# craabreu/openmm-nonbonded-slicing

Hardware: AMD Instinct MI355X
Metric: ns/day (force evaluation only, dt = 2 fs) (higher is better)
Workload: dtype f32

## Files before the change

### openmm-nonbonded-slicing_amd/csrc/engine.hip

```cpp
#include "../../include/snb.h"
#include "snb_internal.h"
#include "switches.h"
#include "host_lists.h"
#include "ewald_fit.h"

#include <algorithm>
#include <cstdio>
#include <cstdlib>
#include <chrono>
#include <cmath>
#include <cstring>
#include <map>
#include <numeric>
#include <set>
#include <thread>
#include <tuple>
#include <type_traits>

namespace snb {

static thread_local std::string g_createError;

static inline void cpuRelax() {
#if defined(__x86_64__) || defined(__i386__)
// ... 902 lines not shown
            if (!noSortGraph && !sortGraphBroken && !cfg.disable_graph && !sortGraphSuspect && !plainSort && N <= (1 << 20)) {
                hipGraphExec_t sortGraphExec = nullptr;
                for (auto& g : sortGraphs) if (g.key.size() == sizeof(key) && std::memcmp(g.key.data(), &key, sizeof(key)) == 0) sortGraphExec = g.exec;
                if (!sortGraphExec) {
                    hipGraph_t graph = nullptr;
                    if (hipStreamBeginCapture(stream, hipStreamCaptureModeThreadLocal) == hipSuccess) {
                        bool threw = false;
                        try { launchNeighborSort<Real>(p, devUserPos, posIsDouble, posStride4, dSortTemp.p, tempBytes, stream); }
                        catch (...) { threw = true; }
                        hipError_t endErr = hipStreamEndCapture(stream, &graph);
                        if (threw) { endErr = hipErrorUnknown; (void)hipGetLastError(); }
                        if (endErr == hipSuccess && graph && hipGraphInstantiate(&sortGraphExec, graph, nullptr, nullptr, 0) == hipSuccess) {
                            SortGraph g; g.key.assign(reinterpret_cast<const unsigned char*>(&key), reinterpret_cast<const unsigned char*>(&key) + sizeof(key)); g.exec = sortGraphExec;
                            if (sortGraphs.size() < 4) sortGraphs.push_back(g);
                            else { (void)hipGraphExecDestroy(sortGraphs[sortGraphVictim].exec); sortGraphs[sortGraphVictim] = g; sortGraphVictim = (sortGraphVictim + 1) % 4; }
                        } else { sortGraphExec = nullptr; sortGraphBroken = true; (void)hipGetLastError(); }
                        if (graph) (void)hipGraphDestroy(graph);
                    } else { sortGraphBroken = true; (void)hipGetLastError(); }
                }
                if (sortGraphExec) { HIPCHECK(hipGraphLaunch(sortGraphExec, stream)); replayed = true; }
            }
            if (!replayed) launchNeighborSort<Real>(p, devUserPos, posIsDouble, posStride4, dSortTemp.p, tempBytes, stream);
        }
        HIPCHECK(hipEventRecord(evRebuild[2], stream));
        const bool predicted = npadPredict > 0 && !sw.nbSyncPadded;
        if (predicted) Npad = npadPredict;
        else {
            int npadDev = 0;
            HIPCHECK(hipMemcpyAsync(&npadDev, dCounters.p + 7, sizeof(int), hipMemcpyDeviceToHost, stream));
            HIPCHECK(hipStreamSynchronize(stream));
            if (npadDev < N || (npadDev & 31)) throw HipError{"neighbour build: inconsistent padded atom count"};
            Npad = npadDev;
        }
        numBlocks = Npad / 32;
        if (Npad >= (1 << SNB_JSHIFT_BITS) - 1) throw HipError{"too many atoms for the 25-bit tile index"};
        posq.resize(Npad); sigeps.resize(Npad); imageOffset.resize((size_t)3 * Npad);
        dSortedToUser.resize(Npad); atomSubset.resize(Npad); atomGrid.resize(Npad); blockSubset.resize(numBlocks);
        layoutForces();
        dBlockCenter.resize((size_t)3 * numBlocks); dBlockHalf.resize((size_t)3 * numBlocks);
        if (tileCap < (size_t)numBlocks * 40) tileCap = (size_t)numBlocks * 40;
        if (tileCap < 64 * 128) tileCap = 64 * 128;
        float sortMs = 0;
        if (!predicted) HIPCHECK(hipEventElapsedTime(&sortMs, evRebuild[0], evRebuild[2]));
        for (int attempt = 0; attempt < 3; attempt++) {
            tileJ.resize(tileCap * 32); tileInfo.resize(tileCap); masks.resize(tileCap * 32); workItems.resize(2 * (tileCap / 4 + 2 * numBlocks + 64)); workItemsStage.resize(tileCap / 4 + 2 * numBlocks + 64); workItemsPartial.resize(tileCap / 4 + 2 * numBlocks + 64);
            p.nPadded = Npad; p.nBlocks = numBlocks; p.blockSubset = blockSubset.p;
            p.shardBegin = shardBegin; p.shardWidth = shardEnd - shardBegin; p.shardPeriod = shardPeriod;
            p.exactPrune = sw.boxPrune ? 0 : 1; p.itemTiles = sw.itemTiles;
            p.blockCenter = dBlockCenter.p; p.blockHalf = dBlockHalf.p;
            p.sortedToUser = dSortedToUser.p; p.userToSorted = dUserToSorted.p; p.posq = posq.p; p.sigeps = sigeps.p; p.imageOffset = imageOffset.p;
            p.atomSubset = atomSubset.p; p.atomGrid = atomGrid.p; p.colRange = colRange.p; p.zIndex = dZIndex.p;
            dAtomCell.resize(Npad); p.atomCell = dAtomCell.p;
            const bool nbTrace = sw.nbTrace;
            if (nbTrace) { dNbTrace.resize((size_t)4 * numBlocks); p.dbgOut = dNbTrace.p; }
            p.tileJ = tileJ.p; p.tileInfo = tileInfo.p; p.masks = masks.p; p.workItems = workItems.p; p.workItemsStage = workItemsStage.p; p.workItemsPartial = workItemsPartial.p; p.counters = dCounters.p;
            p.tileCapacity = (int)tileCap; p.workCapacity = (int)(tileCap / 4 + 2 * numBlocks + 64); p.maskCapacity = (int)tileCap;
            if (!predicted || attempt > 0) HIPCHECK(hipEventRecord(evRebuild[0], stream));
            launchNeighborBuild<Real>(p, stream);
            HIPCHECK(hipEventRecord(evRebuild[1], stream));
            if (sideBuilding) {
                sideSeq = ++nbPubSeq;
                launchNeighborPublish(dCounters.p, dNbPub, sideSeq, stream);
                return true;
            }
            int h[8] = {0, 0, 0, 0, 0, 0, 0, 0};
            if (hNbPub && dNbPub && !sw.nbNoSpin) {
                const int seq = ++nbPubSeq;
                launchNeighborPublish(dCounters.p, dNbPub, seq, stream);
                waitForTotals(seq, h, stream);
                HIPCHECK(hipStreamSynchronize(stream));
            } else {
                HIPCHECK(hipMemcpyAsync(h, dCounters.p, sizeof(h), hipMemcpyDeviceToHost, stream));
                HIPCHECK(hipStreamSynchronize(stream));
            }
            if (!sortGraphSuspect && stats.n_rebuilds > 0 && h[7] > 2 * std::max(Npad, N) && !sideBuilding) {
                sortGraphSuspect = true;
                if (sw.verbose) fprintf(stderr, "[snb] rebuild: padded count %d after %d: phase A once more without its graph\n", h[7], Npad);
                return gpuRebuild();
            }
            if (predicted && (h[7] > Npad || h[7] < N || (h[7] & 31))) {
                if (h[7] < N || (h[7] & 31)) throw HipError{"neighbour build: inconsistent padded atom count"};
                npadPredict = 0; padMispredictions++;
                if (sw.verbose) fprintf(stderr, "[snb] rebuild: padded count %d exceeded the predicted %d, repeating with the exact count (%lld so far)\n", h[7], Npad, (long long)padMispredictions);
                return gpuRebuild();
            }
            if (nbTrace && h[3] == 0) {
                std::vector<long long> tr((size_t)4 * numBlocks);
                HIPCHECK(hipMemcpy(tr.data(), dNbTrace.p, sizeof(long long) * tr.size(), hipMemcpyDeviceToHost));
                long long t0min = tr[0], t1max = tr[1]; std::vector<long long> dur(numBlocks);
                tr.resize((size_t)4 * numBlocks);
                for (int b = 0; b < numBlocks; b++) { t0min = std::min(t0min, tr[2 * b]); t1max = std::max(t1max, tr[2 * b + 1]); dur[b] = tr[2 * b + 1] - tr[2 * b]; }
                std::vector<long long> sorted = dur; std::sort(sorted.begin(), sorted.end());
                fprintf(stderr, "[snb] nb trace: span %.1f us; per-block duration median %.1f us, p90 %.1f, p99 %.1f, max %.1f us; last start at %.1f us\n", (t1max - t0min) / 100.0, sorted[numBlocks / 2] / 100.0,
                        sorted[numBlocks * 9 / 10] / 100.0, sorted[numBlocks * 99 / 100] / 100.0, sorted.back() / 100.0, (t1max - t0min) / 100.0);
                { std::vector<long long> a(numBlocks), b(numBlocks), c(numBlocks);
                  for (int k = 0; k < numBlocks; k++) { a[k] = tr[2 * numBlocks + 2 * k] - tr[2 * k]; b[k] = tr[2 * numBlocks + 2 * k + 1] - tr[2 * numBlocks + 2 * k]; c[k] = tr[2 * k + 1] - tr[2 * numBlocks + 2 * k + 1]; }
                  std::sort(a.begin(), a.end()); std::sort(b.begin(), b.end()); std::sort(c.begin(), c.end());
                  fprintf(stderr, "[snb] nb trace: median prologue %.1f us, gather %.1f us, final flush %.1f us\n", a[numBlocks / 2] / 100.0, b[numBlocks / 2] / 100.0, c[numBlocks / 2] / 100.0); }
                long long lastStart = 0; for (int b = 0; b < numBlocks; b++) lastStart = std::max(lastStart, tr[2 * b] - t0min);
                fprintf(stderr, "[snb] nb trace: last block start %.1f us after the first\n", lastStart / 100.0);
            }
            if (h[3] == 0) { acceptBuild(h, sortMs); gpuBuilt = true; needRebuild = false; paramsDirty = false; stepsSinceRebuild = 0; (void)t0; return true; }
            if (sw.verbose) fprintf(stderr, "[snb] gpu neighbour build attempt %d: tiles %d work %d masks %d overflow %d partial %d maxPartTiles %d maxPartWork %d (cap %zu, region %zu / %zu)\n", attempt, h[0], h[1], h[2], h[3], h[4], h[5], h[6], tileCap, tileCap / 64, (tileCap / 4 + 2 * numBlocks + 64) / 64);
            if ((size_t)h[5] > tileCap / 64 || (size_t)h[6] > (tileCap / 4 + 2 * numBlocks + 64) / 64) { tileCap = std::max((size_t)h[5] * 64 * 5 / 4, tileCap * 3 / 2) + 4096; continue; }
            return false;
        }
        return false;
    }

    void fillPme(PmeParams<Real>& p, PmePlan<Real>& plan, bool wantEnergy, const int* need, bool cellsReady = false, bool trace = false) {
        p.d = plan.d; p.nsub = nGrids; p.natoms = Npad; p.posq = posq.p; p.sigeps = sigeps.p; p.atomSubset = atomSubset.p; p.atomGrid = atomGrid.p;
        p.cells = pmeCells.p;
        if (sw.pmeTrace) { if (!dPmeTrace.p) { dPmeTrace.resize(8); HIPCHECK(hipMemset(dPmeTrace.p, 0, 64)); } p.trace = dPmeTrace.p; }
        p.stepTrace = (trace && plan.dispersion == (cfg.method == SNB_LJPME)) ? dStepTrace.p : nullptr;
        p.cellsReady = (!plan.dispersion && cellsReady) ? 1 : 0;
        p.fixDev = dFixScale.p ? dFixScale.p + (plan.dispersion ? 2 : 0) : nullptr;
        p.gridReal = plan.gridReal.p; p.gridCplx = plan.gridCplx.p; p.planeB = plan.gridCplxB.p; p.planeEterm = plan.planeEtermReady ? plan.planeEterm.p : nullptr; p.twx = plan.twx.p; p.twy = plan.twy.p; p.twz = plan.twz.p;
        p.modx = plan.modx.p; p.mody = plan.mody.p; p.modz = plan.modz.p;
        const double det = box[0] * box[4] * box[8], sc = 1.0 / det;
        const double r[9] = {box[4] * box[8] * sc, 0, 0, -box[3] * box[8] * sc, box[0] * box[8] * sc, 0,
                             (box[3] * box[7] - box[4] * box[6]) * sc, -box[0] * box[7] * sc, box[0] * box[4] * sc};
        for (int i = 0; i < 9; i++) { p.recip[i] = (Real)r[i]; p.recipLo[i] = (Real)(r[i] - (double)p.recip[i]); }
        p.alpha = (Real)plan.alpha; p.volume = (Real)det; p.dispersion = plan.dispersion ? 1 : 0;
        p.lambdas = dLambdas.p; p.sliceNeed = need; p.gridSubset = gridSubset.p; p.nsubTotal = nsub; p.mix = cfg.shard_count == 1 ? 1 : 0;
        p.mix16 = sw.mix16 ? 1 : 0;
        p.sliceE = sliceE.p; p.fpx = fpx.p; p.fpy = fpy.p; p.fpz = fpz.p; p.wantEnergy = wantEnergy ? 1 : 0;
        p.sortNcx = p.sortNcy = 0; p.groupX = p.groupY = 1; p.colRange = nullptr;
        p.zSlabs = 1;
        if (plan.d.nz % 2 == 0 && plan.d.nz >= 32 && !(sizeof(Real) == 4)) p.zSlabs = 2;
        if (sw.zSlabs >= 1 && plan.d.nz % sw.zSlabs == 0) p.zSlabs = sw.zSlabs;
        int ncx, ncy, gx, gy;
        if (brickGeometry(plan, ncx, ncy, gx, gy)) {
            p.sortNcx = ncx; p.sortNcy = ncy; p.groupX = gx; p.groupY = gy; p.colRange = colRange.p;
            p.ownSlabs = plan.ownSlabs; p.ownMargin = plan.ownMargin; p.ownPartial = plan.ownPartial.p; p.ownBusy = plan.ownBusy.p;
            p.strays = plan.strays.p; p.strayCount = dStrayCount.p ? dStrayCount.p + (plan.dispersion ? 1 : 0) : nullptr;
            if (!p.ownPartial || !p.ownBusy || !p.strays || !p.strayCount) p.ownSlabs = 0;
        }
    }
    bool brickGeometry(const PmePlan<Real>& plan, int& ncx, int& ncy, int& gx, int& gy) const {
        if (colCells[0] <= 0) return false;
        ncx = pme.d.nx / colCells[0]; ncy = pme.d.ny / colCells[1];
        const int gMin = sw.brickGroup;
        auto group = [gMin](int n, int ncols) { if (n % ncols) return 0; const int cpc = n / ncols; for (int g = gMin; g <= 4; g++) if (g * cpc >= 5 && ncols % g == 0) return g; return 0; };
        gx = group(plan.d.nx, ncx); gy = group(plan.d.ny, ncy);
        const bool packable = plan.d.nx < 1024 && plan.d.ny < 1024 && plan.d.nz < 1024;
        return packable && gx > 0 && gy > 0 && sizeof(double) * (size_t)(gx * plan.d.nx / ncx) * (gy * plan.d.ny / ncy) * plan.d.nz <= 100 * 1024;
    }
    void planPlaneTable(PmePlan<Real>& plan) {
        if (!plan.planeEterm.p || !plan.gridCplxB.p || nGrids <= 0) { plan.planeEtermReady = false; return; }
        double key[10]; for (int i = 0; i < 9; i++) key[i] = box[i]; key[9] = plan.alpha;
        if (plan.planeEtermReady && plan.planeEtermFilled && std::memcmp(key, plan.planeEtermKey, sizeof(key)) == 0) return;
        std::memcpy(plan.planeEtermKey, key, sizeof(key));
        plan.planeEtermReady = false;
// ... 968 lines not shown
```

### openmm-nonbonded-slicing_amd/csrc/neighbor.hip

```cpp
#include "snb_internal.h"
#include <cstring>
#include <algorithm>
#include <string.h>
#include <rocprim/rocprim.hpp>

namespace snb {

struct Lattice { float ax, bx, by, cx, cy, cz; };
template <typename P> __device__ inline bool useBoxWalk(const P& p) { return p.boxWalk != 0; }
template <typename Real> __device__ inline Lattice latticeOf(const NbParams<Real>& p) {
    return Lattice{(float)p.boxm[0], (float)p.boxm[3], (float)p.boxm[4], (float)p.boxm[6], (float)p.boxm[7], (float)p.boxm[8]};
}
__device__ inline void minImage(float& dx, float& dy, float& dz, const Lattice& L) {
    float s = rintf(dz / L.cz); dx -= s * L.cx; dy -= s * L.cy; dz -= s * L.cz;
    s = rintf(dy / L.by); dx -= s * L.bx; dy -= s * L.by;
    s = rintf(dx / L.ax); dx -= s * L.ax;
}
__device__ inline int orderedInt(float f) { const int i = __float_as_int(f); return i >= 0 ? i : i ^ 0x7FFFFFFF; }
template <typename In> __global__ void k_nbExtent(const In* __restrict__ userPos, int stride, int n, int* __restrict__ ext) {
    const int u = blockIdx.x * blockDim.x + threadIdx.x;
    float lo[3] = {3e38f, 3e38f, 3e38f}, hi[3] = {-3e38f, -3e38f, -3e38f};
    if (u < n) for (int d = 0; d < 3; d++) { const float v = (float)userPos[(size_t)u * stride + d]; lo[d] = v; hi[d] = v; }
#pragma unroll
    for (int o = 32; o > 0; o >>= 1)
// ... 139 lines not shown
    if (b >= p.nBlocks) return;
    const int s = b * 32 + k;
    const bool real = p.sortedToUser[s] >= 0;
    const auto v = p.posq[s];
    float mn[3] = {real ? (float)v.x : 3e38f, real ? (float)v.y : 3e38f, real ? (float)v.z : 3e38f};
    float mx[3] = {real ? (float)v.x : -3e38f, real ? (float)v.y : -3e38f, real ? (float)v.z : -3e38f};
#pragma unroll
    for (int o = 16; o > 0; o >>= 1)
#pragma unroll
        for (int d = 0; d < 3; d++) { mn[d] = fminf(mn[d], __shfl_xor(mn[d], o, 64)); mx[d] = fmaxf(mx[d], __shfl_xor(mx[d], o, 64)); }
    if (k == 0) {
        bool tooWide = false;
        for (int d = 0; d < 3; d++) {
            p.blockCenter[3 * b + d] = 0.5f * (mn[d] + mx[d]); p.blockHalf[3 * b + d] = 0.5f * (mx[d] - mn[d]) + 1e-5f;
            if ((mx[d] - mn[d]) + 2.f * p.listCutoff >= (float)p.boxm[4 * d]) tooWide = true;
        }
        if (tooWide) atomicAdd(&p.counters[3], 1);
    }
}

__device__ inline bool ownsPair(int I, int J) { return ((I + J) & 1) ? (I > J) : (I < J); }
__device__ inline int nbSliceOf(int a, int b) { return a > b ? a * (a + 1) / 2 + b : b * (b + 1) / 2 + a; }
__device__ inline int lanePrefix(unsigned long long m) { return __builtin_amdgcn_mbcnt_hi((unsigned)(m >> 32), __builtin_amdgcn_mbcnt_lo((unsigned)m, 0)); }

constexpr int NB_PARTS = 64;
constexpr int NB_CAP = 768;
constexpr int NB_MAXT = NB_CAP / 32;

template <typename Real> __device__ inline int runLowerBound(const NbParams<Real>& p, int a, int b, float zq, bool asc, int lane) {
    int lo = a, hi = b;
    while (hi > lo) {
        const int len = hi - lo;
        const int step = (len + 63) / 64;
        const int idx = lo + lane * step;
        bool before = false;
        if (idx < hi) { const float z = (float)p.posq[idx].z; before = asc ? (z < zq) : (z > zq); }
        const int nb = __popcll(__ballot(before));
        if (nb == 0) return lo;
        const int newLo = lo + (nb - 1) * step + 1;
        int newHi = lo + nb * step; if (newHi > hi) newHi = hi;
        lo = newLo; hi = newHi;
        if (step == 1) return lo;
    }
    return lo;
}

template <typename Real> __global__ __launch_bounds__(256, 4) void k_nbBuildTiles(const NbParams<Real> p) {
    __shared__ int s_list[4][NB_CAP];
    __shared__ unsigned s_mask[4][NB_MAXT][32];
    __shared__ int s_tileSub[4][NB_MAXT];
    __shared__ int s_query[4][128];
    __shared__ int s_qrow[4][128];
    __shared__ int s_imgI[4][27][5]; __shared__ float s_imgF[4][27][2];
    __shared__ int s_cmb[4][3][64];
    __shared__ float4 s_ipos[4][16]; __shared__ float2 s_iposZ[4][16];
    const int lane = threadIdx.x & 63;
    const int wid = __builtin_amdgcn_readfirstlane(threadIdx.x >> 6);
    const int kOwned = p.nOwned - 1 - (blockIdx.x * 4 + wid);
    if (kOwned < 0) return;
    const int I = (kOwned / p.shardWidth) * p.shardPeriod + p.shardBegin + kOwned % p.shardWidth;
    if (I >= p.nBlocks) return;
    const long long tStart = p.dbgOut ? (long long)wall_clock64() : 0;
    int* list = s_list[wid];
    unsigned (*mask)[32] = s_mask[wid];
    int* tileSub = s_tileSub[wid];
    int* query = s_query[wid];
    int* qrow = s_qrow[wid];
    int* cmbStart = s_cmb[wid][0]; int* cmbPrefix = s_cmb[wid][1]; int* cmbCode = s_cmb[wid][2];
    const float R = p.listCutoff, R2 = R * R;
    const float cxx = p.blockCenter[3 * I], cyy = p.blockCenter[3 * I + 1], czz = p.blockCenter[3 * I + 2];
    const float hx = p.blockHalf[3 * I], hy = p.blockHalf[3 * I + 1], hz = p.blockHalf[3 * I + 2];
    const int il = lane & 31, half = lane >> 5;
    const int uI = p.sortedToUser[I * 32 + il];
    if (__shfl(uI, 0, 64) < 0) return;
    bool failed = false;

    auto flush = [&](int count, bool hasDiag) {
        __builtin_amdgcn_fence(__ATOMIC_RELEASE, "wavefront");
        __builtin_amdgcn_wave_barrier();
        const int nT = count >> 5;
        for (int k = lane; k < nT * 32; k += 64) mask[k >> 5][k & 31] = 0u;
        __builtin_amdgcn_wave_barrier();
        if (hasDiag && half == 0) { unsigned m = 0; for (int j = 0; j <= il; j++) m |= 1u << j; mask[0][il] = m; }
        __builtin_amdgcn_wave_barrier();
        for (int t = half; t < nT; t += 2) {
            const int e = list[t * 32 + il];
            const unsigned long long bal = __ballot(e == -1);
            const unsigned jPad = half ? (unsigned)(bal >> 32) : (unsigned)bal;
            const unsigned row = (uI < 0) ? 0xFFFFFFFFu : jPad;
            if (row) atomicOr(&mask[t][il], row);
        }
        __builtin_amdgcn_wave_barrier();
        int mine[NB_CAP / 64];
#pragma unroll
        for (int r = 0; r < NB_CAP / 64; r++) { const int k2 = lane + 64 * r; const int e = (k2 < count && !(hasDiag && k2 < 32)) ? list[k2] : -1; mine[r] = (e == -1) ? -1 : (e & SNB_JIDX_MASK); }
        auto resolve = [&](int nq) {
            __builtin_amdgcn_fence(__ATOMIC_RELEASE, "wavefront");
            __builtin_amdgcn_wave_barrier();
            for (int qi = 0; qi < nq; qi++) {
                const int target = query[qi], row = qrow[qi];
#pragma unroll
                for (int r = 0; r < NB_CAP / 64; r++)
                    if (mine[r] == target) { const int k2 = lane + 64 * r; atomicOr(&mask[k2 >> 5][row], 1u << (k2 & 31)); }
            }
            __builtin_amdgcn_wave_barrier();
        };
        int nq = 0;
        const int e0 = uI >= 0 ? p.uExclStart[uI] : 0, e1 = uI >= 0 ? p.uExclStart[uI + 1] : 0;
        int maxLen = e1 - e0;
#pragma unroll
        for (int o = 32; o > 0; o >>= 1) { const int other = __shfl_xor(maxLen, o, 64); maxLen = maxLen > other ? maxLen : other; }
        for (int k = 0; k < maxLen; k++) {
            bool want = false; int sp = -1;
            if (half == 0 && e0 + k < e1) {
                sp = p.userToSorted[p.uExclList[e0 + k]];
                const int J = sp >> 5;
                if (J == I) { if (hasDiag) atomicOr(&mask[0][il], 1u << (sp & 31)); }
                else want = ownsPair(I, J);
            }
            const unsigned long long m = __ballot(want);
            const int nNew = __popcll(m);
            if (nq + nNew > 128) { resolve(nq); nq = 0; }
            if (want) { const int o = nq + lanePrefix(m); query[o] = sp; qrow[o] = il; }
            nq += nNew;
        }
        resolve(nq);
        __builtin_amdgcn_fence(__ATOMIC_RELEASE, "wavefront");
        __builtin_amdgcn_wave_barrier();
        int first = 0, w0 = 0, wp = 0;
        const int CH = p.itemTiles;
        const int nFull = nT / CH, nPart = (nT % CH) ? 1 : 0;
        const int part = I & (NB_PARTS - 1);
        int* cnt = p.counters + 32 * (1 + part);
        const int tileRegion = p.tileCapacity / NB_PARTS, workRegion = p.workCapacity / NB_PARTS;
        if (lane == 0) { first = atomicAdd(&cnt[0], nT); w0 = atomicAdd(&cnt[1], nFull); wp = nPart ? atomicAdd(&cnt[4], 1) : 0; }
        first = __builtin_amdgcn_readfirstlane(first); w0 = __builtin_amdgcn_readfirstlane(w0); wp = __builtin_amdgcn_readfirstlane(wp);
        if (first + nT > tileRegion || w0 + nFull > workRegion || wp + nPart > workRegion) { failed = true; return; }
        first += part * tileRegion; w0 += part * workRegion; wp += part * workRegion;
        for (int k = lane; k < count; k += 64) p.tileJ[(size_t)first * 32 + k] = list[k];
        unsigned long long anyBits = 0ull;
        for (int t2 = 0; t2 < nT; t2 += 2) {
            const int t = t2 + half;
            const unsigned row = (t < nT) ? mask[t][il] : 0u;
            const unsigned long long bal = __ballot(row != 0u);
            if ((unsigned)bal) anyBits |= 1ull << t2;
            if ((unsigned)(bal >> 32)) anyBits |= 1ull << (t2 + 1);
        }
        const int nMasked = __popcll(anyBits);
        int mi0 = 0;
        if (nMasked > 0) {
            if (lane == 0) mi0 = atomicAdd(&cnt[2], nMasked);
            mi0 = __builtin_amdgcn_readfirstlane(mi0);
            if (mi0 + nMasked > p.maskCapacity / NB_PARTS) { failed = true; return; }
            mi0 += part * (p.maskCapacity / NB_PARTS);
        }
        for (int t2 = 0; t2 < nT; t2 += 2) {
            const int t = t2 + half;
            if (t < nT && ((anyBits >> t) & 1ull)) p.masks[(size_t)(mi0 + __popcll(anyBits & ((1ull << t) - 1ull))) * 32 + il] = mask[t][il];
        }
        __builtin_amdgcn_fence(__ATOMIC_RELEASE, "wavefront");
        __builtin_amdgcn_wave_barrier();
        const int subIb = p.blockSubset[I];
        for (int t = lane; t < nT; t += 64) p.tileInfo[first + t] = make_int4(nbSliceOf(subIb, tileSub[t]), ((anyBits >> t) & 1ull) ? mi0 + __popcll(anyBits & ((1ull << t) - 1ull)) : -1, tileSub[t], 0);
        const int subI = p.blockSubset[I];
        for (int k = lane; k < nFull; k += 64) p.workItemsStage[w0 + k] = make_int4(I, first + CH * k, CH, subI);
        if (nPart && lane == 0) p.workItemsPartial[wp] = make_int4(I, first + CH * nFull, nT % CH, subI);
        __builtin_amdgcn_wave_barrier();
    };

    const long long tProlog = p.dbgOut ? (long long)wall_clock64() : 0;
    if (lane < 32) { list[lane] = (uI >= 0) ? ((I * 32 + lane) | (SNB_JCODE_CENTER << SNB_JSHIFT_BITS)) : -1; }
    if (lane == 0) tileSub[0] = p.blockSubset[I];
    int count = 32;
    bool hasDiag = true;

    const Lattice Lt = latticeOf(p);
    const float X0 = cxx - hx - R, X1 = cxx + hx + R, Y0 = cyy - hy - R, Y1 = cyy + hy + R, Z0 = czz - hz - R, Z1 = czz + hz + R;
    const float feps = 1e-5f;
    const bool rectCell = Lt.bx == 0.f && Lt.cx == 0.f && Lt.cy == 0.f && !useBoxWalk(p);
    int (*imgI)[5] = s_imgI[wid]; float (*imgF)[2] = s_imgF[wid];
    int nImg = 0;
    for (int img = 0; img < 27; img++) {
        const int kx = img % 3 - 1, ky = (img / 3) % 3 - 1, kz = img / 9 - 1;
        const float tz = kz * Lt.cz, ty = ky * Lt.by + kz * Lt.cy, tx = kx * Lt.ax + ky * Lt.bx + kz * Lt.cx;
        float fz0 = (Z0 - tz) / Lt.cz - feps, fz1 = (Z1 - tz) / Lt.cz + feps;
        if (fz1 < 0.f || fz0 >= 1.f) continue;
        fz0 = fz0 < 0.f ? 0.f : fz0; fz1 = fz1 > 1.f ? 1.f : fz1;
        const float sy0 = fz0 * Lt.cy, sy1 = fz1 * Lt.cy;
        float fy0 = (Y0 - ty - (sy0 > sy1 ? sy0 : sy1)) / Lt.by - feps, fy1 = (Y1 - ty - (sy0 < sy1 ? sy0 : sy1)) / Lt.by + feps;
        if (fy1 < 0.f || fy0 >= 1.f) continue;
        fy0 = fy0 < 0.f ? 0.f : fy0; fy1 = fy1 > 1.f ? 1.f : fy1;
        const float sx0 = fz0 * Lt.cx, sx1 = fz1 * Lt.cx, ux0 = fy0 * Lt.bx, ux1 = fy1 * Lt.bx;
        float fx0 = (X0 - tx - (sx0 > sx1 ? sx0 : sx1) - (ux0 > ux1 ? ux0 : ux1)) / Lt.ax - feps, fx1 = (X1 - tx - (sx0 < sx1 ? sx0 : sx1) - (ux0 < ux1 ? ux0 : ux1)) / Lt.ax + feps;
        if (fx1 < 0.f || fx0 >= 1.f) continue;
        fx0 = fx0 < 0.f ? 0.f : fx0; fx1 = fx1 > 1.f ? 1.f : fx1;
        const int gx0 = (int)(fx0 * p.ncx), gy0 = (int)(fy0 * p.ncy);
        int gx1 = (int)(fx1 * p.ncx), gy1 = (int)(fy1 * p.ncy);
        gx1 = gx1 > p.ncx - 1 ? p.ncx - 1 : gx1; gy1 = gy1 > p.ncy - 1 ? p.ncy - 1 : gy1;
        const int nyc = gy1 - gy0 + 1, ncols = (gx1 - gx0 + 1) * nyc;
        const int code = (kz + 1) * 9 + (ky + 1) * 3 + (kx + 1);
        if (lane == 0) { imgI[nImg][0] = gx0; imgI[nImg][1] = gy0; imgI[nImg][2] = nyc; imgI[nImg][3] = ncols; imgI[nImg][4] = code; imgF[nImg][0] = fz0; imgF[nImg][1] = fz1; }
        nImg++;
    }
    __builtin_amdgcn_fence(__ATOMIC_RELEASE, "wavefront");
    __builtin_amdgcn_wave_barrier();
    float4* ipos = s_ipos[wid]; float2* iposZ = s_iposZ[wid];
    const bool exact = p.exactPrune != 0;
    if (lane < 16) {
        const auto q0 = p.posq[I * 32 + 2 * lane], q1 = p.posq[I * 32 + 2 * lane + 1];
        ipos[lane] = make_float4((float)q0.x, (float)q1.x, (float)q0.y, (float)q1.y); iposZ[lane] = make_float2((float)q0.z, (float)q1.z);
    }
    int filtered = 32;
    auto exactFilter = [&]() {
        __builtin_amdgcn_fence(__ATOMIC_RELEASE, "wavefront");
        __builtin_amdgcn_wave_barrier();
        int out = filtered;
        for (int b0 = filtered; b0 < count; b0 += 64) {
            const int k = b0 + lane;
            bool keep = k < count;
            const int e = keep ? list[k] : 0;
            float px = 0.f, py = 0.f, pz = 0.f;
            if (keep) {
                const int sc = (e >> SNB_JSHIFT_BITS) & 127;
                const int kx = sc / 25 - 2, ky = (sc % 25) / 5 - 2, kz = sc % 5 - 2;
                const auto q = p.posq[e & SNB_JIDX_MASK];
                px = (float)q.x + kx * Lt.ax + ky * Lt.bx + kz * Lt.cx; py = (float)q.y + ky * Lt.by + kz * Lt.cy; pz = (float)q.z + kz * Lt.cz;
            }
            typedef float v2f __attribute__((ext_vector_type(2)));
            float best = 3e38f;
#pragma unroll 8
            for (int a = 0; a < 16; a++) {
                const float4 xy = ipos[a]; const float2 zz = iposZ[a];
                const v2f ddx = v2f{xy.x, xy.y} - px, ddy = v2f{xy.z, xy.w} - py, ddz = v2f{zz.x, zz.y} - pz;
                const v2f d2 = ddx * ddx + ddy * ddy + ddz * ddz;
                best = fminf(best, fminf(d2.x, d2.y));
            }
            keep = keep && best < R2;
            __builtin_amdgcn_wave_barrier();
            const unsigned long long m = __ballot(keep);
            if (keep) { const int o = out + lanePrefix(m); list[o] = e; }
            out += __popcll(m);
        }
        count = out; filtered = out;
        __builtin_amdgcn_fence(__ATOMIC_RELEASE, "wavefront");
        __builtin_amdgcn_wave_barrier();
    };

    for (int s = 0; s < p.nSubsets && !failed; s++) {
        int segStart = count;
        const int2* ranges = p.colRange + (size_t)s * p.ncx * p.ncy;
        const int* zIndex = p.zIndex + (size_t)s * p.ncx * p.ncy * 65;
        int nCmb = 0;

        auto runCandidates = [&]() {
            __builtin_amdgcn_fence(__ATOMIC_RELEASE, "wavefront");
            __builtin_amdgcn_wave_barrier();
            const int len = lane < nCmb ? cmbPrefix[lane] : 0;
            int incl = len;
#pragma unroll
            for (int o = 1; o < 64; o <<= 1) { const int t = __shfl_up(incl, o, 64); if (lane >= o) incl += t; }
            const int total = __shfl(incl, 63, 64);
            __builtin_amdgcn_wave_barrier();
            cmbPrefix[lane] = incl - len;
            __builtin_amdgcn_fence(__ATOMIC_RELEASE, "wavefront");
            __builtin_amdgcn_wave_barrier();
            for (int v0 = 0; v0 < total && !failed; v0 += 64) {
                const int v = v0 + lane;
                bool ok = v < total;
                int j = 0, code = SNB_JCODE_CENTER;
                if (ok) {
                    int k = 0;
#pragma unroll
                    for (int st = 32; st > 0; st >>= 1) if (k + st < 64 && cmbPrefix[k + st] <= v) k += st;
                    const int g = cmbStart[k] + (v - cmbPrefix[k]), cc = cmbCode[k];
                    code = cc & 255;
                    j = ((((g >> 5) << 1) | (cc >> 8)) << 5) | (g & 31);
                }
                if (ok) {
                    int kx = code % 3 - 1, ky = (code / 3) % 3 - 1, kz = code / 9 - 1;
                    const auto q = p.posq[j];
                    const int sc = p.atomCell[j];
                    kx -= (sc & 3) - 1; ky -= ((sc >> 2) & 3) - 1; kz -= ((sc >> 4) & 3) - 1;
                    const float px = (float)q.x + kx * Lt.ax + ky * Lt.bx + kz * Lt.cx, py = (float)q.y + ky * Lt.by + kz * Lt.cy, pz = (float)q.z + kz * Lt.cz;
                    float dx = fabsf(px - cxx) - hx, dy = fabsf(py - cyy) - hy, dz = fabsf(pz - czz) - hz;
                    dx = dx > 0 ? dx : 0; dy = dy > 0 ? dy : 0; dz = dz > 0 ? dz : 0;
                    ok = (dx * dx + dy * dy + dz * dz < R2) && ((float)q.y < 1e8f) && kx >= -2 && kx <= 2 && ky >= -2 && ky <= 2 && kz >= -2 && kz <= 2;
                    code = (kx + 2) * 25 + (ky + 2) * 5 + (kz + 2);
                }
                const unsigned long long m = __ballot(ok);
                const int nNew = __popcll(m);
                if (count + nNew > NB_CAP - 32 && exact) exactFilter();
                if (count + nNew > NB_CAP - 32) {
                    const int padded = (count + 31) & ~31;
                    for (int k = count + lane; k < padded; k += 64) list[k] = -1;
                    for (int t = (segStart >> 5) + lane; t < (padded >> 5); t += 64) tileSub[t] = s;
                    flush(padded, hasDiag);
                    hasDiag = false; count = 0; segStart = 0; filtered = 0;
                }
                if (ok) { const int o = count + lanePrefix(m); list[o] = j | (code << SNB_JSHIFT_BITS); }
                count += nNew;
            }
            __builtin_amdgcn_wave_barrier();
            nCmb = 0;
        };

        for (int im = 0; im < nImg && !failed; im++) {
            const int gx0 = imgI[im][0], gy0 = imgI[im][1], nyc = imgI[im][2], ncols = imgI[im][3], code = imgI[im][4];
            const float fz0 = imgF[im][0], fz1 = imgF[im][1];
            for (int c0 = 0; c0 < ncols && !failed; c0 += 64) {
                const int c = c0 + lane;
                int cStart = 0, cLen = 0;
                if (c < ncols) {
                    const int ccx = gx0 + c / nyc, ccy = gy0 + c % nyc;
                    const int col = ccx * p.ncy + ccy;
                    const int2 rg = ranges[col];
                    if (rg.y > rg.x) {
                        const int serp = ccx * p.ncy + ((ccx & 1) ? (p.ncy - 1 - ccy) : ccy);
                        float fa = fz0, fb = fz1;
                        if (rectCell) {
                            const int kx = code % 3 - 1, ky = (code / 3) % 3 - 1, kz = code / 9 - 1;
                            const float wx = Lt.ax / p.ncx, wy = Lt.by / p.ncy, slack = 1e-5f * (Lt.ax + Lt.by);
                            const float xlo = ccx * wx + kx * Lt.ax - slack, xhi = (ccx + 1) * wx + kx * Lt.ax + slack;
                            const float ylo = ccy * wy + ky * Lt.by - slack, yhi = (ccy + 1) * wy + ky * Lt.by + slack;
                            float ddx = fmaxf(0.f, fmaxf(xlo - (cxx + hx), (cxx - hx) - xhi)), ddy = fmaxf(0.f, fmaxf(ylo - (cyy + hy), (cyy - hy) - yhi));
                            const float rz2 = R2 - ddx * ddx - ddy * ddy;
                            if (rz2 <= 0.f) { fa = 1.f; fb = 0.f; }
                            else {
                                const float rz = sqrtf(rz2) * 1.0001f;
                                const float za = (czz - hz - rz - kz * Lt.cz) / Lt.cz - feps, zb = (czz + hz + rz - kz * Lt.cz) / Lt.cz + feps;
                                fa = fmaxf(fa, za); fb = fminf(fb, zb);
                            }
                        }
                        if (fb > fa) {
                        if (serp & 1) { const float t = 1.f - fb; fb = 1.f - fa; fa = t; }
                        int blo = ((int)(fa * 1048575.0f) >> 14) - 1, bhi = ((int)(fb * 1048575.0f) >> 14) + 1;
                        blo = blo < 0 ? 0 : blo; bhi = bhi > 63 ? 63 : bhi;
                        const int* zi = zIndex + (size_t)col * 65;
                        cStart = zi[blo]; cLen = zi[bhi + 1] - zi[blo];
                        }
                    }
                }
#pragma unroll
                for (int part = 0; part < 2; part++) {
                    const int pi = part == 0 ? ((I & 1) ^ 1) : (I & 1);
                    int a = cStart, b = cStart + cLen;
                    if (part == 0) b = b < I * 32 ? b : I * 32; else a = a > (I + 1) * 32 ? a : (I + 1) * 32;
                    auto compact = [pi](int x) { const int B = x >> 5; return (((B + 1 - pi) >> 1) << 5) + (((B & 1) == pi) ? (x & 31) : 0); };
                    const int g0 = b > a ? compact(a) : 0, gLen = b > a ? compact(b) - g0 : 0;
                    const unsigned long long mq = __ballot(gLen > 0);
                    const int nQ = __popcll(mq);
                    if (nQ == 0) continue;
                    if (nCmb + nQ > 64) runCandidates();
                    if (gLen > 0) { const int o = nCmb + lanePrefix(mq); cmbStart[o] = g0; cmbPrefix[o] = gLen; cmbCode[o] = code | (pi << 8); }
                    nCmb += nQ;
                }
            }
        }
        if (nCmb > 0 && !failed) runCandidates();
        if (exact && !failed) exactFilter();
        const int padded = (count + 31) & ~31;
        for (int k = count + lane; k < padded; k += 64) list[k] = -1;
        for (int t = (segStart >> 5) + lane; t < (padded >> 5); t += 64) tileSub[t] = s;
        count = padded; filtered = padded;
    }
    const long long tGather = p.dbgOut ? (long long)wall_clock64() : 0;
    if (!failed && count > 0) flush(count, hasDiag);
    if (failed && lane == 0) atomicAdd(&p.counters[3], 1);
    if (p.dbgOut && lane == 0) { p.dbgOut[2 * I] = tStart; p.dbgOut[2 * I + 1] = (long long)wall_clock64(); p.dbgOut[2 * p.nBlocks + 2 * I] = tProlog; p.dbgOut[2 * p.nBlocks + 2 * I + 1] = tGather; }
}

template <typename Real> __global__ void k_nbClear(const NbParams<Real> p) {
    const size_t i = (size_t)blockIdx.x * blockDim.x + threadIdx.x;
    const size_t nCols = (size_t)p.nSubsets * p.ncx * p.ncy;
    if (i < 7 || (i >= 32 && i < (size_t)32 * (1 + NB_PARTS))) p.counters[i] = 0;
    if (i < nCols) p.colRange[i] = make_int2(0x7FFFFFFF, 0);
    if (i < nCols * 65) p.zIndex[i] = 0x7F7F7F7F;
    if (i < (size_t)p.nPadded) p.sortedToUser[i] = -1;
}

template <typename Real> __global__ __launch_bounds__(256) void k_nbCompactWork(const NbParams<Real> p) {
    __shared__ int s_off[2][NB_PARTS + 1];
    if (threadIdx.x == 0) {
        int accF = 0, accP = 0, tiles = 0, masksN = 0, maxTiles = 0, maxWork = 0;
        for (int q = 0; q < NB_PARTS; q++) {
            const int* c = p.counters + 32 * (1 + q);
            s_off[0][q] = accF; s_off[1][q] = accP;
            accF += c[1]; accP += c[4]; tiles += c[0]; masksN += c[2];
            maxTiles = maxTiles > c[0] ? maxTiles : c[0]; maxTiles = maxTiles > c[2] ? maxTiles : c[2];
            maxWork = maxWork > c[1] ? maxWork : c[1]; maxWork = maxWork > c[4] ? maxWork : c[4];
        }
        s_off[0][NB_PARTS] = accF; s_off[1][NB_PARTS] = accP;
        if (blockIdx.x == 0) { p.counters[0] = tiles; p.counters[1] = accF; p.counters[2] = masksN; p.counters[4] = accP; p.counters[5] = maxTiles; p.counters[6] = maxWork; }
    }
    __syncthreads();
    const int q = blockIdx.x % NB_PARTS, which = blockIdx.x / NB_PARTS;
    const int workRegion = p.workCapacity / NB_PARTS;
    const int n = s_off[which][q + 1] - s_off[which][q];
    const int4* src = (which ? p.workItemsPartial : p.workItemsStage) + (size_t)q * workRegion;
    int4* dst = p.workItems + (which ? s_off[0][NB_PARTS] : 0) + s_off[which][q];
    if (n > workRegion) return;
    if ((size_t)(dst - p.workItems) + (size_t)n > (size_t)2 * p.workCapacity) return;
    for (int i = threadIdx.x; i < n; i += 256) dst[i] = src[i];
}

template <typename Real> size_t nbSortTempBytes(int n) {
    size_t bytes = 0, b2 = 0, b3 = 0;
    unsigned long long* k = nullptr; int* v = nullptr;
    (void)rocprim::radix_sort_pairs(nullptr, bytes, k, k, v, v, (size_t)n, 0, 64, (hipStream_t)0);
    (void)rocprim::inclusive_scan(nullptr, b2, v, v, (size_t)n, rocprim::maximum<int>(), (hipStream_t)0);
    (void)rocprim::exclusive_scan(nullptr, b3, v, v, 0, (size_t)n, rocprim::plus<int>(), (hipStream_t)0);
    return std::max(bytes, std::max(b2, b3));
}

template <typename Real> void launchNeighborSort(const NbParams<Real>& p, const void* userPos, int isDouble, int stride4, void* sortTemp, size_t sortTempBytes, hipStream_t s) {
    const int n = p.nAtoms;
    const int stride = stride4 ? 4 : 3;
    dim3 block(256), gridN((n + 255) / 256);
    launchZeroFill(p.counters, sizeof(int) * 32 * (1 + NB_PARTS), s);
    if (n <= 0) return;
    if (isDouble) hipLaunchKernelGGL((k_nbKeys<Real, double>), gridN, block, 0, s, p, (const double*)userPos, stride);
    else hipLaunchKernelGGL((k_nbKeys<Real, float>), gridN, block, 0, s, p, (const float*)userPos, stride);
// ... 53 lines not shown
```

Baseline: 496.6.

## Streamline neighbour-build kernel: cheaper candidate lookup, mask init, and integer math

Reworks the neighbour-list build kernel. Candidate runs are packed into int2 with precomputed offsets and pre-decoded image codes, and each lane finds its run with ballots and readlane instead of a shared-memory binary search. Mask rows are written directly instead of being zeroed and then atomically ORed. Divisions and modulos are replaced by multiply-shift or reciprocal arithmetic, and exclusion handling is spread across both half-waves. It also nests the 27-image loop to hoist work and adds finer per-phase trace timers, which adds complexity and some risk of correctness bugs in the decoding tricks.

```diff
diff --git a/openmm-nonbonded-slicing_amd/csrc/engine.hip b/openmm-nonbonded-slicing_amd/csrc/engine.hip
--- a/openmm-nonbonded-slicing_amd/csrc/engine.hip
+++ b/openmm-nonbonded-slicing_amd/csrc/engine.hip
@@ -978,7 +978,7 @@
             p.atomSubset = atomSubset.p; p.atomGrid = atomGrid.p; p.colRange = colRange.p; p.zIndex = dZIndex.p;
             dAtomCell.resize(Npad); p.atomCell = dAtomCell.p;
             const bool nbTrace = sw.nbTrace;
-            if (nbTrace) { dNbTrace.resize((size_t)4 * numBlocks); p.dbgOut = dNbTrace.p; }
+            if (nbTrace) { dNbTrace.resize((size_t)8 * numBlocks); launchZeroFill(dNbTrace.p, sizeof(long long) * 8 * (size_t)numBlocks, stream); p.dbgOut = dNbTrace.p; }
             p.tileJ = tileJ.p; p.tileInfo = tileInfo.p; p.masks = masks.p; p.workItems = workItems.p; p.workItemsStage = workItemsStage.p; p.workItemsPartial = workItemsPartial.p; p.counters = dCounters.p;
             p.tileCapacity = (int)tileCap; p.workCapacity = (int)(tileCap / 4 + 2 * numBlocks + 64); p.maskCapacity = (int)tileCap;
             if (!predicted || attempt > 0) HIPCHECK(hipEventRecord(evRebuild[0], stream));
@@ -1011,20 +1011,30 @@
                 return gpuRebuild();
             }
             if (nbTrace && h[3] == 0) {
-                std::vector<long long> tr((size_t)4 * numBlocks);
+                std::vector<long long> tr((size_t)8 * numBlocks);
                 HIPCHECK(hipMemcpy(tr.data(), dNbTrace.p, sizeof(long long) * tr.size(), hipMemcpyDeviceToHost));
-                long long t0min = tr[0], t1max = tr[1]; std::vector<long long> dur(numBlocks);
-                tr.resize((size_t)4 * numBlocks);
-                for (int b = 0; b < numBlocks; b++) { t0min = std::min(t0min, tr[2 * b]); t1max = std::max(t1max, tr[2 * b + 1]); dur[b] = tr[2 * b + 1] - tr[2 * b]; }
-                std::vector<long long> sorted = dur; std::sort(sorted.begin(), sorted.end());
-                fprintf(stderr, "[snb] nb trace: span %.1f us; per-block duration median %.1f us, p90 %.1f, p99 %.1f, max %.1f us; last start at %.1f us\n", (t1max - t0min) / 100.0, sorted[numBlocks / 2] / 100.0,
-                        sorted[numBlocks * 9 / 10] / 100.0, sorted[numBlocks * 99 / 100] / 100.0, sorted.back() / 100.0, (t1max - t0min) / 100.0);
-                { std::vector<long long> a(numBlocks), b(numBlocks), c(numBlocks);
-                  for (int k = 0; k < numBlocks; k++) { a[k] = tr[2 * numBlocks + 2 * k] - tr[2 * k]; b[k] = tr[2 * numBlocks + 2 * k + 1] - tr[2 * numBlocks + 2 * k]; c[k] = tr[2 * k + 1] - tr[2 * numBlocks + 2 * k + 1]; }
-                  std::sort(a.begin(), a.end()); std::sort(b.begin(), b.end()); std::sort(c.begin(), c.end());
-                  fprintf(stderr, "[snb] nb trace: median prologue %.1f us, gather %.1f us, final flush %.1f us\n", a[numBlocks / 2] / 100.0, b[numBlocks / 2] / 100.0, c[numBlocks / 2] / 100.0); }
-                long long lastStart = 0; for (int b = 0; b < numBlocks; b++) lastStart = std::max(lastStart, tr[2 * b] - t0min);
-                fprintf(stderr, "[snb] nb trace: last block start %.1f us after the first\n", lastStart / 100.0);
+                long long t0min = 0, t1max = 0, lastStart = 0; bool any = false;
+                std::vector<long long> ph[7];
+                double sum[7] = {0, 0, 0, 0, 0, 0, 0};
+                for (int b = 0; b < numBlocks; b++) {
+                    const long long* o = &tr[8 * (size_t)b];
+                    if (o[1] <= o[0] || o[0] == 0) continue;
+                    if (!any) { t0min = o[0]; t1max = o[1]; any = true; }
+                    t0min = std::min(t0min, o[0]); t1max = std::max(t1max, o[1]); lastStart = std::max(lastStart, o[0]);
+                    const long long innerFlush = o[6] - (o[1] - o[3]);
+                    const long long v[7] = {o[1] - o[0], o[2] - o[0], o[3] - o[2], o[4], o[5], o[6], (o[3] - o[2]) - o[4] - o[5] - innerFlush};
+                    for (int k = 0; k < 7; k++) { ph[k].push_back(v[k]); sum[k] += (double)v[k]; }
+                }
+                if (any) {
+                    for (auto& v : ph) std::sort(v.begin(), v.end());
+                    const size_t nb = ph[0].size();
+                    fprintf(stderr, "[snb] nb trace: span %.1f us; per-block duration median %.1f us, p90 %.1f, p99 %.1f, max %.1f us; last block start %.1f us after the first\n", (t1max - t0min) / 100.0,
+                            ph[0][nb / 2] / 100.0, ph[0][nb * 9 / 10] / 100.0, ph[0][nb * 99 / 100] / 100.0, ph[0].back() / 100.0, (lastStart - t0min) / 100.0);
+                    fprintf(stderr, "[snb] nb trace: median prologue %.1f us, gather %.1f us (run queueing %.1f, candidate walk %.1f, exact filter %.1f), flushes %.1f us\n",
+                            ph[1][nb / 2] / 100.0, ph[2][nb / 2] / 100.0, ph[6][nb / 2] / 100.0, ph[3][nb / 2] / 100.0, ph[4][nb / 2] / 100.0, ph[5][nb / 2] / 100.0);
+                    fprintf(stderr, "[snb] nb trace: share of the blocks' time: prologue %.3f, run queueing %.3f, candidate walk %.3f, exact filter %.3f, flushes %.3f (%zu blocks)\n",
+                            sum[1] / sum[0], sum[6] / sum[0], sum[3] / sum[0], sum[4] / sum[0], sum[5] / sum[0], nb);
+                }
             }
             if (h[3] == 0) { acceptBuild(h, sortMs); gpuBuilt = true; needRebuild = false; paramsDirty = false; stepsSinceRebuild = 0; (void)t0; return true; }
             if (sw.verbose) fprintf(stderr, "[snb] gpu neighbour build attempt %d: tiles %d work %d masks %d overflow %d partial %d maxPartTiles %d maxPartWork %d (cap %zu, region %zu / %zu)\n", attempt, h[0], h[1], h[2], h[3], h[4], h[5], h[6], tileCap, tileCap / 64, (tileCap / 4 + 2 * numBlocks + 64) / 64);
diff --git a/openmm-nonbonded-slicing_amd/csrc/neighbor.hip b/openmm-nonbonded-slicing_amd/csrc/neighbor.hip
--- a/openmm-nonbonded-slicing_amd/csrc/neighbor.hip
+++ b/openmm-nonbonded-slicing_amd/csrc/neighbor.hip
@@ -215,7 +215,7 @@
     __shared__ int s_query[4][128];
     __shared__ int s_qrow[4][128];
     __shared__ int s_imgI[4][27][5]; __shared__ float s_imgF[4][27][2];
-    __shared__ int s_cmb[4][3][64];
+    __shared__ int s_cmbPrefix[4][64]; __shared__ int2 s_cmbRun[4][64];
     __shared__ float4 s_ipos[4][16]; __shared__ float2 s_iposZ[4][16];
     const int lane = threadIdx.x & 63;
     const int wid = __builtin_amdgcn_readfirstlane(threadIdx.x >> 6);
@@ -223,13 +223,16 @@
     if (kOwned < 0) return;
     const int I = (kOwned / p.shardWidth) * p.shardPeriod + p.shardBegin + kOwned % p.shardWidth;
     if (I >= p.nBlocks) return;
-    const long long tStart = p.dbgOut ? (long long)wall_clock64() : 0;
+    const bool trace = p.dbgOut != nullptr;
+    auto now = [trace]() { return trace ? (long long)wall_clock64() : 0ll; };
+    const long long tStart = now();
+    long long tkWalk = 0, tkExact = 0, tkFlush = 0;
     int* list = s_list[wid];
     unsigned (*mask)[32] = s_mask[wid];
     int* tileSub = s_tileSub[wid];
     int* query = s_query[wid];
     int* qrow = s_qrow[wid];
-    int* cmbStart = s_cmb[wid][0]; int* cmbPrefix = s_cmb[wid][1]; int* cmbCode = s_cmb[wid][2];
+    int* cmbPrefix = s_cmbPrefix[wid]; int2* cmbRun = s_cmbRun[wid];
     const float R = p.listCutoff, R2 = R * R;
     const float cxx = p.blockCenter[3 * I], cyy = p.blockCenter[3 * I + 1], czz = p.blockCenter[3 * I + 2];
     const float hx = p.blockHalf[3 * I], hy = p.blockHalf[3 * I + 1], hz = p.blockHalf[3 * I + 2];
@@ -239,19 +242,17 @@
     bool failed = false;
 
     auto flush = [&](int count, bool hasDiag) {
+        const long long tf0 = now();
         __builtin_amdgcn_fence(__ATOMIC_RELEASE, "wavefront");
         __builtin_amdgcn_wave_barrier();
         const int nT = count >> 5;
-        for (int k = lane; k < nT * 32; k += 64) mask[k >> 5][k & 31] = 0u;
-        __builtin_amdgcn_wave_barrier();
-        if (hasDiag && half == 0) { unsigned m = 0; for (int j = 0; j <= il; j++) m |= 1u << j; mask[0][il] = m; }
-        __builtin_amdgcn_wave_barrier();
         for (int t = half; t < nT; t += 2) {
             const int e = list[t * 32 + il];
             const unsigned long long bal = __ballot(e == -1);
             const unsigned jPad = half ? (unsigned)(bal >> 32) : (unsigned)bal;
-            const unsigned row = (uI < 0) ? 0xFFFFFFFFu : jPad;
-            if (row) atomicOr(&mask[t][il], row);
+            unsigned row = (uI < 0) ? 0xFFFFFFFFu : jPad;
+            if (hasDiag && t == 0) row |= (2u << il) - 1u;
+            mask[t][il] = row;
         }
         __builtin_amdgcn_wave_barrier();
         int mine[NB_CAP / 64];
@@ -273,9 +274,10 @@
         int maxLen = e1 - e0;
 #pragma unroll
         for (int o = 32; o > 0; o >>= 1) { const int other = __shfl_xor(maxLen, o, 64); maxLen = maxLen > other ? maxLen : other; }
-        for (int k = 0; k < maxLen; k++) {
+        for (int k0 = 0; k0 < maxLen; k0 += 2) {
+            const int k = k0 + half;
             bool want = false; int sp = -1;
-            if (half == 0 && e0 + k < e1) {
+            if (e0 + k < e1) {
                 sp = p.userToSorted[p.uExclList[e0 + k]];
                 const int J = sp >> 5;
                 if (J == I) { if (hasDiag) atomicOr(&mask[0][il], 1u << (sp & 31)); }
@@ -317,9 +319,11 @@
             if (mi0 + nMasked > p.maskCapacity / NB_PARTS) { failed = true; return; }
             mi0 += part * (p.maskCapacity / NB_PARTS);
         }
+        int nBefore = 0;
         for (int t2 = 0; t2 < nT; t2 += 2) {
-            const int t = t2 + half;
-            if (t < nT && ((anyBits >> t) & 1ull)) p.masks[(size_t)(mi0 + __popcll(anyBits & ((1ull << t) - 1ull))) * 32 + il] = mask[t][il];
+            const int b0 = (int)((anyBits >> t2) & 1ull), b1 = (int)((anyBits >> (t2 + 1)) & 1ull);
+            if (half ? b1 : b0) p.masks[(size_t)(mi0 + nBefore + (half ? b0 : 0)) * 32 + il] = mask[t2 + half][il];
+            nBefore += b0 + b1;
         }
         __builtin_amdgcn_fence(__ATOMIC_RELEASE, "wavefront");
         __builtin_amdgcn_wave_barrier();
@@ -329,9 +333,9 @@
         for (int k = lane; k < nFull; k += 64) p.workItemsStage[w0 + k] = make_int4(I, first + CH * k, CH, subI);
         if (nPart && lane == 0) p.workItemsPartial[wp] = make_int4(I, first + CH * nFull, nT % CH, subI);
         __builtin_amdgcn_wave_barrier();
+        tkFlush += now() - tf0;
     };
 
-    const long long tProlog = p.dbgOut ? (long long)wall_clock64() : 0;
     if (lane < 32) { list[lane] = (uI >= 0) ? ((I * 32 + lane) | (SNB_JCODE_CENTER << SNB_JSHIFT_BITS)) : -1; }
     if (lane == 0) tileSub[0] = p.blockSubset[I];
     int count = 32;
@@ -343,27 +347,40 @@
     const bool rectCell = Lt.bx == 0.f && Lt.cx == 0.f && Lt.cy == 0.f && !useBoxWalk(p);
     int (*imgI)[5] = s_imgI[wid]; float (*imgF)[2] = s_imgF[wid];
     int nImg = 0;
-    for (int img = 0; img < 27; img++) {
-        const int kx = img % 3 - 1, ky = (img / 3) % 3 - 1, kz = img / 9 - 1;
-        const float tz = kz * Lt.cz, ty = ky * Lt.by + kz * Lt.cy, tx = kx * Lt.ax + ky * Lt.bx + kz * Lt.cx;
+#pragma nounroll
+    for (int kz = -1; kz <= 1; kz++) {
+        const float tz = kz * Lt.cz;
         float fz0 = (Z0 - tz) / Lt.cz - feps, fz1 = (Z1 - tz) / Lt.cz + feps;
         if (fz1 < 0.f || fz0 >= 1.f) continue;
         fz0 = fz0 < 0.f ? 0.f : fz0; fz1 = fz1 > 1.f ? 1.f : fz1;
         const float sy0 = fz0 * Lt.cy, sy1 = fz1 * Lt.cy;
-        float fy0 = (Y0 - ty - (sy0 > sy1 ? sy0 : sy1)) / Lt.by - feps, fy1 = (Y1 - ty - (sy0 < sy1 ? sy0 : sy1)) / Lt.by + feps;
-        if (fy1 < 0.f || fy0 >= 1.f) continue;
-        fy0 = fy0 < 0.f ? 0.f : fy0; fy1 = fy1 > 1.f ? 1.f : fy1;
-        const float sx0 = fz0 * Lt.cx, sx1 = fz1 * Lt.cx, ux0 = fy0 * Lt.bx, ux1 = fy1 * Lt.bx;
-        float fx0 = (X0 - tx - (sx0 > sx1 ? sx0 : sx1) - (ux0 > ux1 ? ux0 : ux1)) / Lt.ax - feps, fx1 = (X1 - tx - (sx0 < sx1 ? sx0 : sx1) - (ux0 < ux1 ? ux0 : ux1)) / Lt.ax + feps;
-        if (fx1 < 0.f || fx0 >= 1.f) continue;
-        fx0 = fx0 < 0.f ? 0.f : fx0; fx1 = fx1 > 1.f ? 1.f : fx1;
-        const int gx0 = (int)(fx0 * p.ncx), gy0 = (int)(fy0 * p.ncy);
-        int gx1 = (int)(fx1 * p.ncx), gy1 = (int)(fy1 * p.ncy);
-        gx1 = gx1 > p.ncx - 1 ? p.ncx - 1 : gx1; gy1 = gy1 > p.ncy - 1 ? p.ncy - 1 : gy1;
-        const int nyc = gy1 - gy0 + 1, ncols = (gx1 - gx0 + 1) * nyc;
-        const int code = (kz + 1) * 9 + (ky + 1) * 3 + (kx + 1);
-        if (lane == 0) { imgI[nImg][0] = gx0; imgI[nImg][1] = gy0; imgI[nImg][2] = nyc; imgI[nImg][3] = ncols; imgI[nImg][4] = code; imgF[nImg][0] = fz0; imgF[nImg][1] = fz1; }
-        nImg++;
+        const float sx0 = fz0 * Lt.cx, sx1 = fz1 * Lt.cx;
+#pragma nounroll
+        for (int ky = -1; ky <= 1; ky++) {
+            const float ty = ky * Lt.by + kz * Lt.cy;
+            float fy0 = (Y0 - ty - (sy0 > sy1 ? sy0 : sy1)) / Lt.by - feps, fy1 = (Y1 - ty - (sy0 < sy1 ? sy0 : sy1)) / Lt.by + feps;
+            if (fy1 < 0.f || fy0 >= 1.f) continue;
+            fy0 = fy0 < 0.f ? 0.f : fy0; fy1 = fy1 > 1.f ? 1.f : fy1;
+            const float ux0 = fy0 * Lt.bx, ux1 = fy1 * Lt.bx;
+            const int gy0 = (int)(fy0 * p.ncy);
+            int gy1 = (int)(fy1 * p.ncy);
+            gy1 = gy1 > p.ncy - 1 ? p.ncy - 1 : gy1;
+            const int nyc = gy1 - gy0 + 1;
+#pragma nounroll
+            for (int kx = -1; kx <= 1; kx++) {
+                const float tx = kx * Lt.ax + ky * Lt.bx + kz * Lt.cx;
+                float fx0 = (X0 - tx - (sx0 > sx1 ? sx0 : sx1) - (ux0 > ux1 ? ux0 : ux1)) / Lt.ax - feps, fx1 = (X1 - tx - (sx0 < sx1 ? sx0 : sx1) - (ux0 < ux1 ? ux0 : ux1)) / Lt.ax + feps;
+                if (fx1 < 0.f || fx0 >= 1.f) continue;
+                fx0 = fx0 < 0.f ? 0.f : fx0; fx1 = fx1 > 1.f ? 1.f : fx1;
+                const int gx0 = (int)(fx0 * p.ncx);
+                int gx1 = (int)(fx1 * p.ncx);
+                gx1 = gx1 > p.ncx - 1 ? p.ncx - 1 : gx1;
+                const int ncols = (gx1 - gx0 + 1) * nyc;
+                const int code = (kz + 1) * 9 + (ky + 1) * 3 + (kx + 1);
+                if (lane == 0) { imgI[nImg][0] = gx0; imgI[nImg][1] = gy0; imgI[nImg][2] = nyc; imgI[nImg][3] = ncols; imgI[nImg][4] = code; imgF[nImg][0] = fz0; imgF[nImg][1] = fz1; }
+                nImg++;
+            }
+        }
     }
     __builtin_amdgcn_fence(__ATOMIC_RELEASE, "wavefront");
     __builtin_amdgcn_wave_barrier();
@@ -374,7 +391,9 @@
         ipos[lane] = make_float4((float)q0.x, (float)q1.x, (float)q0.y, (float)q1.y); iposZ[lane] = make_float2((float)q0.z, (float)q1.z);
     }
     int filtered = 32;
+    const long long tProlog = now();
     auto exactFilter = [&]() {
+        const long long te0 = now();
         __builtin_amdgcn_fence(__ATOMIC_RELEASE, "wavefront");
         __builtin_amdgcn_wave_barrier();
         int out = filtered;
@@ -385,7 +404,8 @@
             float px = 0.f, py = 0.f, pz = 0.f;
             if (keep) {
                 const int sc = (e >> SNB_JSHIFT_BITS) & 127;
-                const int kx = sc / 25 - 2, ky = (sc % 25) / 5 - 2, kz = sc % 5 - 2;
+                const int c25 = (sc * 41) >> 10, r25 = sc - 25 * c25, c5 = (r25 * 13) >> 6;
+                const int kx = c25 - 2, ky = c5 - 2, kz = r25 - 5 * c5 - 2;
                 const auto q = p.posq[e & SNB_JIDX_MASK];
                 px = (float)q.x + kx * Lt.ax + ky * Lt.bx + kz * Lt.cx; py = (float)q.y + ky * Lt.by + kz * Lt.cy; pz = (float)q.z + kz * Lt.cz;
             }
@@ -407,6 +427,7 @@
         count = out; filtered = out;
         __builtin_amdgcn_fence(__ATOMIC_RELEASE, "wavefront");
         __builtin_amdgcn_wave_barrier();
+        tkExact += now() - te0;
     };
 
     for (int s = 0; s < p.nSubsets && !failed; s++) {
@@ -416,38 +437,46 @@
         int nCmb = 0;
 
         auto runCandidates = [&]() {
+            const long long tw0 = now(), nested0 = tkExact + tkFlush;
             __builtin_amdgcn_fence(__ATOMIC_RELEASE, "wavefront");
             __builtin_amdgcn_wave_barrier();
             const int len = lane < nCmb ? cmbPrefix[lane] : 0;
             int incl = len;
 #pragma unroll
             for (int o = 1; o < 64; o <<= 1) { const int t = __shfl_up(incl, o, 64); if (lane >= o) incl += t; }
-            const int total = __shfl(incl, 63, 64);
-            __builtin_amdgcn_wave_barrier();
-            cmbPrefix[lane] = incl - len;
+            const int total = __builtin_amdgcn_readfirstlane(__shfl(incl, 63, 64));
+            {
+                const int2 run = lane < nCmb ? cmbRun[lane] : make_int2(0, 0);
+                const int c27 = run.y & 255;
+                const int rz = (c27 * 57) >> 9, r9 = c27 - 9 * rz, ry = (r9 * 11) >> 5, rx = r9 - 3 * ry;
+                __builtin_amdgcn_wave_barrier();
+                cmbPrefix[lane] = lane < nCmb ? incl - len : 0x7FFFFFFF;
+                cmbRun[lane] = make_int2(run.x - (incl - len), rx | (ry << 2) | (rz << 4) | (run.y & 256));
+            }
             __builtin_amdgcn_fence(__ATOMIC_RELEASE, "wavefront");
             __builtin_amdgcn_wave_barrier();
             for (int v0 = 0; v0 < total && !failed; v0 += 64) {
                 const int v = v0 + lane;
                 bool ok = v < total;
                 int j = 0, code = SNB_JCODE_CENTER;
-                if (ok) {
-                    int k = 0;
-#pragma unroll
-                    for (int st = 32; st > 0; st >>= 1) if (k + st < 64 && cmbPrefix[k + st] <= v) k += st;
-                    const int g = cmbStart[k] + (v - cmbPrefix[k]), cc = cmbCode[k];
-                    code = cc & 255;
-                    j = ((((g >> 5) << 1) | (cc >> 8)) << 5) | (g & 31);
+                {
+                    const int pre = cmbPrefix[lane];
+                    const int ka = __popcll(__ballot(pre <= v0)) - 1, kb = __popcll(__ballot(pre <= v0 + 63)) - 1;
+                    int k = ka;
+                    for (int r = ka + 1; r <= kb; r++) k += (v >= __builtin_amdgcn_readlane(pre, r)) ? 1 : 0;
+                    const int2 run = cmbRun[k];
+                    const int g = run.x + v;
+                    j = ((((g >> 5) << 1) | (run.y >> 8)) << 5) | (g & 31);
+                    code = run.y;
                 }
                 if (ok) {
-                    int kx = code % 3 - 1, ky = (code / 3) % 3 - 1, kz = code / 9 - 1;
                     const auto q = p.posq[j];
                     const int sc = p.atomCell[j];
-                    kx -= (sc & 3) - 1; ky -= ((sc >> 2) & 3) - 1; kz -= ((sc >> 4) & 3) - 1;
+                    const int kx = (code & 3) - (sc & 3), ky = ((code >> 2) & 3) - ((sc >> 2) & 3), kz = ((code >> 4) & 3) - ((sc >> 4) & 3);
                     const float px = (float)q.x + kx * Lt.ax + ky * Lt.bx + kz * Lt.cx, py = (float)q.y + ky * Lt.by + kz * Lt.cy, pz = (float)q.z + kz * Lt.cz;
                     float dx = fabsf(px - cxx) - hx, dy = fabsf(py - cyy) - hy, dz = fabsf(pz - czz) - hz;
                     dx = dx > 0 ? dx : 0; dy = dy > 0 ? dy : 0; dz = dz > 0 ? dz : 0;
-                    ok = (dx * dx + dy * dy + dz * dz < R2) && ((float)q.y < 1e8f) && kx >= -2 && kx <= 2 && ky >= -2 && ky <= 2 && kz >= -2 && kz <= 2;
+                    ok = (dx * dx + dy * dy + dz * dz < R2) && ((float)q.y < 1e8f) && (sc & (sc >> 1) & 0x15) == 0;
                     code = (kx + 2) * 25 + (ky + 2) * 5 + (kz + 2);
                 }
                 const unsigned long long m = __ballot(ok);
@@ -465,16 +494,20 @@
             }
             __builtin_amdgcn_wave_barrier();
             nCmb = 0;
+            tkWalk += (now() - tw0) - (tkExact + tkFlush - nested0);
         };
 
         for (int im = 0; im < nImg && !failed; im++) {
             const int gx0 = imgI[im][0], gy0 = imgI[im][1], nyc = imgI[im][2], ncols = imgI[im][3], code = imgI[im][4];
             const float fz0 = imgF[im][0], fz1 = imgF[im][1];
+            const float rnyc = 1.0f / (float)nyc;
             for (int c0 = 0; c0 < ncols && !failed; c0 += 64) {
                 const int c = c0 + lane;
                 int cStart = 0, cLen = 0;
                 if (c < ncols) {
-                    const int ccx = gx0 + c / nyc, ccy = gy0 + c % nyc;
+                    int cq = (int)(((float)c + 0.5f) * rnyc), cr = c - cq * nyc;
+                    if (cr < 0) { cq--; cr += nyc; } else if (cr >= nyc) { cq++; cr -= nyc; }
+                    const int ccx = gx0 + cq, ccy = gy0 + cr;
                     const int col = ccx * p.ncy + ccy;
                     const int2 rg = ranges[col];
                     if (rg.y > rg.x) {
@@ -514,7 +547,7 @@
                     const int nQ = __popcll(mq);
                     if (nQ == 0) continue;
                     if (nCmb + nQ > 64) runCandidates();
-                    if (gLen > 0) { const int o = nCmb + lanePrefix(mq); cmbStart[o] = g0; cmbPrefix[o] = gLen; cmbCode[o] = code | (pi << 8); }
+                    if (gLen > 0) { const int o = nCmb + lanePrefix(mq); cmbRun[o] = make_int2(g0, code | (pi << 8)); cmbPrefix[o] = gLen; }
                     nCmb += nQ;
                 }
             }
@@ -526,10 +559,13 @@
         for (int t = (segStart >> 5) + lane; t < (padded >> 5); t += 64) tileSub[t] = s;
         count = padded; filtered = padded;
     }
-    const long long tGather = p.dbgOut ? (long long)wall_clock64() : 0;
+    const long long tGather = now();
     if (!failed && count > 0) flush(count, hasDiag);
     if (failed && lane == 0) atomicAdd(&p.counters[3], 1);
-    if (p.dbgOut && lane == 0) { p.dbgOut[2 * I] = tStart; p.dbgOut[2 * I + 1] = (long long)wall_clock64(); p.dbgOut[2 * p.nBlocks + 2 * I] = tProlog; p.dbgOut[2 * p.nBlocks + 2 * I + 1] = tGather; }
+    if (trace && lane == 0) {
+        long long* o = p.dbgOut + 8 * (size_t)I;
+        o[0] = tStart; o[1] = now(); o[2] = tProlog; o[3] = tGather; o[4] = tkWalk; o[5] = tkExact; o[6] = tkFlush; o[7] = 0;
+    }
 }
 
 template <typename Real> __global__ void k_nbClear(const NbParams<Real> p) {
```

Result: no change. 500.2 (median of 6 runs) (+0.7%).
